# bcsefercik/markerless-robot-camera-calibration

Measured on AMD Instinct MI355X. Metric: point-cloud frames/sec at 200k pts/frame, higher is better.
Workload: dtype f32

## Files before the change

### markerless-robot-camera-calibration_amd/csrc/sv_conv.hip

```cpp
#include <stdarg.h>
#include <stdio.h>
#include <stdlib.h>
#include <vector>

#include "sv_conv_params.h"

namespace sv {

static thread_local char g_last_instance[128] = "";
static thread_local double g_want_scale_override = -1.0;
static thread_local double g_tail_override = -1.0;
void note_instance(const char* fmt, ...) {
  va_list ap;
  va_start(ap, fmt);
  vsnprintf(g_last_instance, sizeof(g_last_instance), fmt, ap);
  va_end(ap);
}
#ifndef SV_CONV_WANT_SCALE_DEFAULT
#define SV_CONV_WANT_SCALE_DEFAULT 0.3
#endif
#ifndef SV_CONV_TAIL_DEFAULT
#define SV_CONV_TAIL_DEFAULT 0.15
#endif
constexpr int chunk_for(int tm, int waves_n) {
// ... 482 lines not shown
  const int rc = launch_traced(q, grid.x, TM_, WAVES_N, NT, stream, [&] {
    if (F && fast && full) {
      if (ring)
        hipLaunchKernelGGL((conv_fwd_kernel<TM_, WAVES_N, NT, F, CPO, (Cfg::PFD > 1), (F && Cfg::USE_FULL)>), grid, dim3(256), lds, stream, q);
      else
        hipLaunchKernelGGL((conv_fwd_kernel<TM_, WAVES_N, NT, F, CPO, false, (F && Cfg::USE_FULL)>), grid, dim3(256), lds, stream, q);
    } else if (F && fast) {
      if (ring)
        hipLaunchKernelGGL((conv_fwd_kernel<TM_, WAVES_N, NT, F, CPO, (Cfg::PFD > 1)>), grid, dim3(256), lds, stream, q);
      else
        hipLaunchKernelGGL((conv_fwd_kernel<TM_, WAVES_N, NT, F, CPO, false>), grid, dim3(256), lds, stream, q);
    } else {
      if (ring)
        hipLaunchKernelGGL((conv_fwd_kernel<TM_, WAVES_N, NT, false, CPO, (Cfg::PFD > 1)>), grid, dim3(256), lds, stream, q);
      else
        hipLaunchKernelGGL((conv_fwd_kernel<TM_, WAVES_N, NT, false, CPO, false>), grid, dim3(256), lds, stream, q);
    }
  });
  if (rc != SV_OK) return rc;
  {
    const bool f = F && fast;
    if (CPO)
      note_instance("conv_fwd_kernel<%d, %d, %d, fused %d>|fast=%d,ring=%d,full=%d", TM_, WAVES_N, NT, CPO, (int)f, (int)ring,
                    (int)(f && full));
    else
      note_instance("conv_fwd_kernel<%d, %d, %d>|fast=%d,ring=%d,full=%d", TM_, WAVES_N, NT, (int)f, (int)ring, (int)(f && full));
  }
  return SV_OK;
}

template <int TM_, int TAIL_TM, int WAVES_N, int NT>
static int launch_conv_dual(const ConvParams& p, hipStream_t stream, double tail_fraction) {
  using Main = ConvCfg<TM_, WAVES_N, NT, 0>;
  using Tail = ConvCfg<TAIL_TM, WAVES_N, NT, 0>;
  const bool fast = p.vec_a && p.buf_ok && (p.Cout % Main::TN == 0);
  const int n128 = (int)(p.Vpad / PLAN_TILE);
  const int tail128 = (int)(n128 * tail_fraction);
  if (!fast || !p.tile_order || tail128 < 1 || tail128 >= n128) return SV_ERR_INVALID;
  ConvParams q = p;
  q.ny = p.Cout / Main::TN;
  q.main_tiles128 = n128 - tail128;
  q.main_blocks = q.main_tiles128 * (PLAN_TILE / TM_) * q.ny;
  q.ntiles = (int)(p.Vpad / TM_);
  const unsigned grid = (unsigned)(q.main_blocks + tail128 * (PLAN_TILE / TAIL_TM) * q.ny);
  const size_t lds = Main::lds_bytes(p.K) > Tail::lds_bytes(p.K) ? Main::lds_bytes(p.K) : Tail::lds_bytes(p.K);
  const int rc = launch_traced(q, grid, TM_, WAVES_N, NT, stream, [&] {
    hipLaunchKernelGGL((conv_fwd_dual_kernel<TM_, TAIL_TM, WAVES_N, NT, true>), dim3(grid), dim3(256), lds, stream, q);
  });
  if (rc != SV_OK) return rc;
  note_instance("conv_fwd_dual_kernel<%d, %d, %d, %d>|fast=1,ring=0,full=0", TM_, TAIL_TM, WAVES_N, NT);
  return SV_OK;
}

struct Candidate {
  int tm, wn, nt;
  int64_t want;
  int cpo;
};

template <int TM_, int WAVES_N, int NT, int CPO = 0>
static bool try_launch(const Candidate& c, const ConvParams& p, hipStream_t stream, int& rc) {
  if (c.tm == TM_ && c.wn == WAVES_N && c.nt == NT && c.cpo == CPO) {
    rc = launch_conv<TM_, WAVES_N, NT, CPO>(p, stream);
    return true;
  }
  return false;
}

static int launch_candidate(const Candidate& c, const ConvParams& p, hipStream_t stream) {
  int rc = SV_ERR_INVALID;
  if (try_launch<128, 4, 3>(c, p, stream, rc) || try_launch<128, 2, 3>(c, p, stream, rc) ||
      try_launch<128, 1, 3>(c, p, stream, rc) || try_launch<64, 4, 3>(c, p, stream, rc) ||
      try_launch<64, 2, 3>(c, p, stream, rc) || try_launch<64, 1, 3>(c, p, stream, rc) ||
      try_launch<32, 4, 3>(c, p, stream, rc) || try_launch<32, 2, 3>(c, p, stream, rc) ||
      try_launch<16, 4, 3>(c, p, stream, rc) ||
      try_launch<128, 4, 2>(c, p, stream, rc) || try_launch<128, 2, 2>(c, p, stream, rc) ||
      try_launch<128, 1, 2>(c, p, stream, rc) || try_launch<64, 4, 2>(c, p, stream, rc) ||
      try_launch<64, 2, 2>(c, p, stream, rc) || try_launch<64, 1, 2>(c, p, stream, rc) ||
      try_launch<32, 4, 2>(c, p, stream, rc) || try_launch<32, 2, 2>(c, p, stream, rc) ||
      try_launch<16, 4, 2>(c, p, stream, rc) ||
      try_launch<64, 4, 1>(c, p, stream, rc) || try_launch<32, 4, 1>(c, p, stream, rc) ||
      try_launch<16, 4, 1>(c, p, stream, rc) || try_launch<128, 2, 1>(c, p, stream, rc) ||
      try_launch<64, 2, 1>(c, p, stream, rc) || try_launch<32, 2, 1>(c, p, stream, rc) ||
      try_launch<128, 1, 1>(c, p, stream, rc) || try_launch<64, 1, 1>(c, p, stream, rc) ||
      try_launch<64, 2, 1, 3>(c, p, stream, rc) || try_launch<32, 2, 1, 3>(c, p, stream, rc) ||
      try_launch<64, 2, 1, 32>(c, p, stream, rc) || try_launch<32, 2, 1, 32>(c, p, stream, rc) ||
      try_launch<32, 4, 1, 32>(c, p, stream, rc) || try_launch<16, 4, 1, 32>(c, p, stream, rc) ||
      try_launch<32, 4, 1, 64>(c, p, stream, rc) || try_launch<16, 4, 1, 64>(c, p, stream, rc))
    return rc;
  set_error("sv_conv_fwd: no kernel instance <%d,%d,%d> cpo %d", c.tm, c.wn, c.nt, c.cpo);
  return SV_ERR_INVALID;
}

static int64_t candidate_wgs(const Candidate& c, const ConvParams& p) {
  const int tn = c.wn * c.nt * 16;
  return (p.Vpad / c.tm) * ((p.Cout + tn - 1) / tn);
}

static int select_and_launch(const ConvParams& p, hipStream_t stream) {
  static const Candidate wide3[] = {{64, 4, 3, 2500}, {32, 4, 3, 1500}, {32, 2, 3, 0}};
  static const Candidate wide3_128[] = {{64, 4, 3, 2500}, {64, 4, 2, 1200}, {32, 4, 3, 1200}, {16, 4, 3, 0}};
  static const Candidate wide3_128_full[] = {{64, 4, 3, 2500}, {32, 4, 3, 1200}, {16, 4, 3, 0}};
  static const Candidate wide2[] = {{128, 4, 2, 1300}, {64, 4, 2, 1500}, {32, 4, 2, 1500}, {32, 2, 2, 0}};
  static const Candidate wide2_64[] = {{128, 4, 2, 1300}, {64, 4, 2, 1500}, {32, 4, 2, 1500}, {16, 4, 1, 0}};
  static const Candidate c64[] = {{64, 4, 1, 1500}, {32, 4, 1, 1500}, {16, 4, 1, 0}};
  static const Candidate c32[] = {{128, 2, 1, 1500}, {64, 2, 1, 1500}, {32, 2, 1, 0}};
  static const Candidate c16[] = {{128, 1, 1, 600}, {64, 1, 1, 0}};
  const Candidate* list;
  int n;
  const int Cout = p.Cout;
  if (Cout > 128 && (Cout % 192 == 0 || Cout % 96 == 0 || Cout > 2048)) {
    if (Cout % 128 != 0) { list = wide3; n = 3; }
    else if (p.Cin % 128 == 0 && p.vec_a) { list = wide3_128_full; n = 3; }
    else { list = wide3_128; n = 4; }
  }
  else if (Cout > 64) { list = Cout % 64 == 0 ? wide2_64 : wide2; n = 4; }
  else if (Cout > 32) { list = c64; n = 3; }
  else if (Cout > 16) { list = c32; n = 3; }
  else { list = c16; n = 2; }
  static const Candidate f3[] = {{64, 2, 1, 3000, 3}, {32, 2, 1, 0, 3}};
  static const Candidate f32_32[] = {{64, 2, 1, 3000, 32}, {32, 2, 1, 0, 32}};
  static const Candidate f32_64[] = {{32, 4, 1, 1500, 32}, {16, 4, 1, 0, 32}};
  static const Candidate f64_64[] = {{32, 4, 1, 1500, 64}, {16, 4, 1, 0, 64}};
  if (p.K > 1) {
    if (p.Cin == 3 && Cout > 16 && Cout <= 32) { list = f3; n = 2; }
    else if (p.Cin == 32 && p.vec_a && Cout == 32) { list = f32_32; n = 2; }
    else if (p.Cin == 32 && p.vec_a && Cout == 64) { list = f32_64; n = 2; }
    else if (p.Cin == 64 && p.vec_a && (Cout == 64 || Cout == 128)) { list = f64_64; n = 2; }
  }
  if (const char* f = getenv("SV_CONV_FORCE_RANGE")) {
    long long vmin = 0, vmax = 0;
    int cout = 0;
    Candidate c = {0, 0, 0, 0, 0};
    if (sscanf(f, "%lld:%lld:%d:%d,%d,%d", &vmin, &vmax, &cout, &c.tm, &c.wn, &c.nt) == 6 && p.Vpad >= vmin && p.Vpad <= vmax &&
        p.Cout == cout && p.K > 1)
      return launch_candidate(c, p, stream);
  }
  if (const char* f = getenv("SV_CONV_FORCE_DENSE")) {
    long long vmin = 0;
    int cout = 0;
    Candidate c = {0, 0, 0, 0, 0};
    if (sscanf(f, "%lld:%d:%d,%d,%d", &vmin, &cout, &c.tm, &c.wn, &c.nt) == 5 && p.Vpad >= vmin && p.Cout == cout && p.K == 1)
      return launch_candidate(c, p, stream);
  }
  if (const char* f = getenv("SV_CONV_FORCE")) {
    Candidate c = {0, 0, 0, 0, 0};
    if (sscanf(f, "%d,%d,%d,%d", &c.tm, &c.wn, &c.nt, &c.cpo) >= 3) return launch_candidate(c, p, stream);
  }
  static const double want_scale =
      getenv("SV_CONV_WANT_SCALE") ? atof(getenv("SV_CONV_WANT_SCALE")) : SV_CONV_WANT_SCALE_DEFAULT;
  static const double tail_fraction = getenv("SV_CONV_TAIL") ? atof(getenv("SV_CONV_TAIL")) : SV_CONV_TAIL_DEFAULT;
  const double ws = g_want_scale_override >= 0.0 ? g_want_scale_override : want_scale;
  const double tf = g_tail_override >= 0.0 ? g_tail_override : tail_fraction;
  for (int i = 0; i < n; ++i)
    if ((double)candidate_wgs(list[i], p) >= ws * (double)list[i].want) {
      const Candidate& c = list[i];
      if (c.tm == 64 && c.wn == 4 && c.nt == 3 && c.cpo == 0 && tf > 0.0 &&
          launch_conv_dual<64, 32, 4, 3>(p, stream, tf) == SV_OK)
        return SV_OK;
      return launch_candidate(c, p, stream);
    }
  return launch_candidate(list[n - 1], p, stream);
}

}

using namespace sv;

extern "C" const char* sv_conv_last_instance(void) { return sv::g_last_instance; }

extern "C" int sv_conv_set_dispatch(double want_scale, double tail_fraction) {
  SV_CHECK_ARG(tail_fraction < 1.0, "tail_fraction must be below 1");
  sv::g_want_scale_override = want_scale;
  sv::g_tail_override = tail_fraction;
  return SV_OK;
}

extern "C" int sv_conv_fwd(const float* in, int64_t V_in, int64_t in_ld, int Cin, const float* W, int K, int Cout,
                           const int32_t* perm, const int32_t* nbr_s, const uint32_t* submask,
                           const int32_t* tile_order, int64_t V_out, int64_t Vpad, const float* scale, const float* shift, const float* residual, int64_t res_ld,
                           int act, float slope, float* out, int64_t out_ld, sv_stream_t stream_) {
  return sv_conv_fwd_acc(in, V_in, in_ld, Cin, W, K, Cout, perm, nbr_s, submask, tile_order, V_out, Vpad, nullptr, 0, scale, shift,
                         residual, res_ld, act, slope, out, out_ld, stream_);
}

extern "C" int sv_conv_fwd_acc(const float* in, int64_t V_in, int64_t in_ld, int Cin, const float* W, int K, int Cout,
                               const int32_t* perm, const int32_t* nbr_s, const uint32_t* submask, const int32_t* tile_order,
                               int64_t V_out, int64_t Vpad, const float* acc_init, int64_t acc_ld, const float* scale,
                               const float* shift, const float* residual, int64_t res_ld, int act, float slope, float* out,
                               int64_t out_ld, sv_stream_t stream_) {
  hipStream_t stream = (hipStream_t)stream_;
  SV_CHECK_ARG(!acc_init || acc_ld >= Cout, "acc_init stride too small");
  SV_CHECK_ARG(Cin > 0 && Cout > 0 && K >= 1 && K <= 32, "bad channel / kernel volume");
  SV_CHECK_ARG(V_out >= 0 && Vpad >= V_out && Vpad % PLAN_TILE == 0, "Vpad must be a multiple of 128 >= V_out");
  SV_CHECK_ARG(in_ld >= Cin && out_ld >= Cout, "row strides too small");
  SV_CHECK_ARG(act >= SV_ACT_NONE && act <= SV_ACT_LEAKY_RELU, "bad activation");
  if (V_out == 0) return SV_OK;
  SV_CHECK_ARG(in && W && out, "null pointer");
  SV_CHECK_ARG(V_in >= 1, "V_in = rows of `in` (every index of the plan is below it)");
  const bool has_plan = perm || nbr_s || submask;
  SV_CHECK_ARG(!has_plan || (perm && nbr_s && submask), "perm, nbr_s and submask must be given together");
  SV_CHECK_ARG(has_plan || K == 1, "K > 1 needs a plan");
  SV_CHECK_ARG(!residual || res_ld >= Cout, "residual stride too small");
  ConvParams p;
  p.in = in; p.in_ld = in_ld; p.Cin = Cin; p.W = W; p.K = K; p.Cout = Cout;
  p.perm = perm; p.nbr_s = nbr_s; p.submask = submask; p.tile_order = tile_order; p.V_out = V_out; p.Vpad = Vpad;
  p.scale = scale; p.shift = shift; p.residual = residual; p.res_ld = res_ld;
  p.acc_init = acc_init; p.acc_ld = acc_ld;
  p.act = act; p.slope = slope; p.out = out; p.out_ld = out_ld;
  p.vec_a = (in_ld % 4 == 0) && (Cin % 4 == 0) && (((uintptr_t)in & 15) == 0);
  const uint64_t in_bytes = ((uint64_t)(V_in - 1) * (uint64_t)in_ld + (uint64_t)Cin) * 4u;
  const uint64_t w_bytes = (uint64_t)K * (uint64_t)Cin * (uint64_t)Cout * 4u;
  const uint64_t out_bytes = ((uint64_t)(V_out - 1) * (uint64_t)out_ld + (uint64_t)Cout) * 4u;
  const uint64_t res_bytes = residual ? ((uint64_t)(V_out - 1) * (uint64_t)res_ld + (uint64_t)Cout) * 4u : 0u;
  const uint64_t acc_bytes = acc_init ? ((uint64_t)(V_out - 1) * (uint64_t)acc_ld + (uint64_t)Cout) * 4u : 0u;
  p.buf_ok = in_bytes < BUF_LIMIT && w_bytes < BUF_LIMIT && out_bytes < BUF_LIMIT && res_bytes < BUF_LIMIT &&
             acc_bytes < BUF_LIMIT && (((uintptr_t)perm & 15) == 0);
  p.acc_bytes = p.buf_ok ? (uint32_t)acc_bytes : 0u;
  if (!p.buf_ok && !has_plan && K == 1 && w_bytes < BUF_LIMIT) {
    int64_t ld_max = in_ld > out_ld ? in_ld : out_ld;
    if (residual && res_ld > ld_max) ld_max = res_ld;
    const int64_t rows = (int64_t)((BUF_LIMIT - 4096u) / ((uint64_t)ld_max * 4u)) / PLAN_TILE * PLAN_TILE;
    if (rows >= PLAN_TILE && rows < V_out) {
      for (int64_t r0 = 0; r0 < V_out; r0 += rows) {
        const int64_t n = V_out - r0 < rows ? V_out - r0 : rows;
        const int rc = sv_conv_fwd_acc(in + r0 * in_ld, n, in_ld, Cin, W, K, Cout, nullptr, nullptr, nullptr, nullptr, n,
                                       (n + PLAN_TILE - 1) / PLAN_TILE * PLAN_TILE, acc_init ? acc_init + r0 * acc_ld : nullptr,
                                       acc_ld, scale, shift, residual ? residual + r0 * res_ld : nullptr, res_ld, act, slope,
                                       out + r0 * out_ld, out_ld, stream_);
        if (rc != SV_OK) return rc;
      }
      return SV_OK;
    }
  }
  p.in_bytes = p.buf_ok ? (uint32_t)in_bytes : 0u;
  p.w_bytes = p.buf_ok ? (uint32_t)w_bytes : 0u;
  p.out_bytes = p.buf_ok ? (uint32_t)out_bytes : 0u;
  p.res_bytes = p.buf_ok ? (uint32_t)res_bytes : 0u;
  p.ntiles = 0;
  p.ny = 0;
  p.trace = nullptr;
  p.main_blocks = 0;
  p.main_tiles128 = 0;
  if (has_plan && K > 1 && K <= 27 && Cin == 3 && Cout == 32 && !acc_init) {
    if (p.buf_ok) return launch_conv_first_mfma(p, stream);
    return launch_conv_first_layer(p, stream);
  }
  if (has_plan && K > 1 && K <= 32 && Cin == 32 && Cout == 32 && p.vec_a && p.buf_ok && !acc_init)
    return launch_conv_thin(p, stream, sv::g_want_scale_override >= 1.0);
  if (!has_plan && K == 1 && Cout <= 4 && p.vec_a && Cin >= 64 && !acc_init) return launch_linear_narrow(p, stream);
  return select_and_launch(p, stream);
}
```

### markerless-robot-camera-calibration_amd/csrc/sv_conv_params.h

```cpp
#pragma once
#include <type_traits>

#include "sv_common.h"

namespace sv {

typedef float f32x4 __attribute__((ext_vector_type(4)));

struct ConvParams {
  const float* in;
  int64_t in_ld;
  int Cin;
  const float* W;
  int K;
  int Cout;
  const int32_t* perm;
  const int32_t* nbr_s;
  const uint32_t* submask;
  const int32_t* tile_order;
  int64_t V_out;
  int64_t Vpad;
  const float* scale;
  const float* shift;
  const float* residual;
  int64_t res_ld;
  const float* acc_init;
  int64_t acc_ld;
  uint32_t acc_bytes;
  int act;
  float slope;
  float* out;
  int64_t out_ld;
  int vec_a;
  uint32_t in_bytes, w_bytes, out_bytes, res_bytes;
  int buf_ok;
  int ntiles;
  int ny;
  unsigned long long* trace;
  int main_blocks;
  int main_tiles128;
};

constexpr int PLAN_TILE = SV_TILE_ROWS;
void note_instance(const char* fmt, ...);
int launch_conv_first_mfma(const ConvParams& p, hipStream_t stream);
int launch_conv_first_layer(const ConvParams& p, hipStream_t stream);
int launch_conv_thin(const ConvParams& p, hipStream_t stream, bool alone);
int launch_linear_narrow(const ConvParams& p, hipStream_t stream);

constexpr uint32_t BUF_ABSENT = 0x80000000u;
constexpr uint32_t BUF_LIMIT = 0x7fff0000u;
typedef int i32x4_t __attribute__((ext_vector_type(4)));
typedef int i32x3_t __attribute__((ext_vector_type(3)));
typedef int i32x2_t __attribute__((ext_vector_type(2)));
template <int N>
__device__ __forceinline__ auto buffer_load_floats(__amdgpu_buffer_rsrc_t rsrc, uint32_t voffset, uint32_t soffset) {
  typedef float vec_t __attribute__((ext_vector_type(N)));
  if constexpr (N == 1) {
    vec_t r;
    r[0] = __builtin_bit_cast(float, __builtin_amdgcn_raw_buffer_load_b32(rsrc, voffset, soffset, 0));
    return r;
  } else if constexpr (N == 2) {
    return __builtin_bit_cast(vec_t, __builtin_amdgcn_raw_buffer_load_b64(rsrc, voffset, soffset, 0));
  } else if constexpr (N == 3) {
    return __builtin_bit_cast(vec_t, __builtin_amdgcn_raw_buffer_load_b96(rsrc, voffset, soffset, 0));
  } else {
    static_assert(N == 4, "1..4 floats per load");
    return __builtin_bit_cast(vec_t, __builtin_amdgcn_raw_buffer_load_b128(rsrc, voffset, soffset, 0));
  }
}

template <int MR>
__device__ __forceinline__ void load_perm_rows(const ConvParams& p, const int64_t rows0, const int lq, int (&o)[MR][4]) {
#pragma unroll
  for (int s = 0; s < MR; ++s) {
    const int64_t r = rows0 + s * 16 + lq * 4;
    if (p.perm) {
      const int4 o4 = *(const int4*)(p.perm + r);
      o[s][0] = o4.x;
      o[s][1] = o4.y;
      o[s][2] = o4.z;
      o[s][3] = o4.w;
    } else {
#pragma unroll
      for (int reg = 0; reg < 4; ++reg) o[s][reg] = (r + reg < p.V_out) ? (int)(r + reg) : -1;
    }
  }
}

template <int MR, int NT, bool PRELOADED = false>
__device__ __forceinline__ void epilogue_buffered(const ConvParams& p, const f32x4 (&acc)[MR][NT], const int64_t rows0,
                                                  const int lq, const int col0, const int (*o_pre)[4] = nullptr) {
  typedef float yvec_t __attribute__((ext_vector_type(NT)));
  const __amdgpu_buffer_rsrc_t rsrc_out = __builtin_amdgcn_make_buffer_rsrc((void*)p.out, 0, (int)p.out_bytes, 0x00020000);
  const __amdgpu_buffer_rsrc_t rsrc_res =
      __builtin_amdgcn_make_buffer_rsrc((void*)p.residual, 0, p.residual ? (int)p.res_bytes : 0, 0x00020000);
  int o[MR][4];
  if constexpr (PRELOADED) {
#pragma unroll
    for (int s = 0; s < MR; ++s)
#pragma unroll
      for (int reg = 0; reg < 4; ++reg) o[s][reg] = o_pre[s][reg];
  } else {
    load_perm_rows<MR>(p, rows0, lq, o);
  }
  float scf[NT], shf[NT];
#pragma unroll
  for (int n = 0; n < NT; ++n) {
    scf[n] = p.scale ? p.scale[col0 + n] : 1.0f;
    shf[n] = p.shift ? p.shift[col0 + n] : (p.scale ? 0.0f : -0.0f);
  }
  const float slope = p.slope;
  auto finish = [&](auto act_tag) {
    constexpr int ACT = decltype(act_tag)::value;
#pragma unroll
    for (int s = 0; s < MR; ++s) {
      yvec_t res[4];
#pragma unroll
      for (int reg = 0; reg < 4; ++reg)
#pragma unroll
        for (int n = 0; n < NT; ++n) res[reg][n] = -0.0f;
      if (p.residual) {
#pragma unroll
        for (int reg = 0; reg < 4; ++reg)
          res[reg] = buffer_load_floats<NT>(
              rsrc_res, o[s][reg] >= 0 ? (uint32_t)o[s][reg] * (uint32_t)(p.res_ld * 4) + (uint32_t)col0 * 4u : BUF_ABSENT,
              0u);
      }
#pragma unroll
      for (int reg = 0; reg < 4; ++reg) {
        yvec_t y;
#pragma unroll
        for (int n = 0; n < NT; ++n) {
          float v = __builtin_fmaf(acc[s][n][reg], scf[n], shf[n]) + res[reg][n];
          if constexpr (ACT == SV_ACT_RELU)
            v = v < 0.f ? 0.f : v;
          else if constexpr (ACT == SV_ACT_LEAKY_RELU)
            v = v > 0.f ? v : v * slope;
          y[n] = v;
        }
        const uint32_t off =
            o[s][reg] >= 0 ? (uint32_t)o[s][reg] * (uint32_t)(p.out_ld * 4) + (uint32_t)col0 * 4u : BUF_ABSENT;
        if constexpr (NT == 1)
          __builtin_amdgcn_raw_buffer_store_b32(__builtin_bit_cast(int, y[0]), rsrc_out, off, 0, 0);
        else if constexpr (NT == 2)
          __builtin_amdgcn_raw_buffer_store_b64(__builtin_bit_cast(i32x2_t, y), rsrc_out, off, 0, 0);
        else if constexpr (NT == 3)
          __builtin_amdgcn_raw_buffer_store_b96(__builtin_bit_cast(i32x3_t, y), rsrc_out, off, 0, 0);
        else
          __builtin_amdgcn_raw_buffer_store_b128(__builtin_bit_cast(i32x4_t, y), rsrc_out, off, 0, 0);
      }
    }
  };
  if (p.act == SV_ACT_RELU)
    finish(std::integral_constant<int, SV_ACT_RELU>{});
  else if (p.act == SV_ACT_LEAKY_RELU)
    finish(std::integral_constant<int, SV_ACT_LEAKY_RELU>{});
  else
    finish(std::integral_constant<int, SV_ACT_NONE>{});
}

}
```

### markerless-robot-camera-calibration_amd/nn.py

```python
import math
from ctypes import c_float, c_int, c_int64, c_size_t

import numpy as np
import torch
import torch.nn as nn

from . import _lib, profiling
from ._lib import SV_ACT_LEAKY_RELU, SV_ACT_NONE, SV_ACT_RELU, call, ptr, stream_ptr
from .sparse import SparseTensor, SplitPlan

KERNEL_OFFSET_PERMUTATION = None

import os as _os


def _parse_split_rules(text):
    rules = []
    for part in text.split(";"):
        if part.strip():
            rows, _, cuts = part.partition(":")
            cuts = tuple(int(v) for v in cuts.split(",") if v)
            rules.append((int(rows), cuts[0] if len(cuts) == 1 else cuts))
    return sorted(rules, key=lambda r: -r[0])


SPLIT_RULES = _parse_split_rules(_os.environ.get("MRCC_SPLIT_RULES", "20000:9,18"))
SPLIT_MIN_CHANNELS = int(_os.environ.get("MRCC_SPLIT_MIN_CHANNELS", "128"))


SPLIT_RULES_ONE_FRAME = _parse_split_rules(_os.environ.get("MRCC_SPLIT_RULES_ONE_FRAME", "50000:9,18"))


def split_points_for(rows):
    for min_rows, cuts in SPLIT_RULES:
        if rows >= min_rows:
            return cuts
    return None


def conv_forward(feats, weight3, plan, V_out, scale=None, shift=None, residual=None, act=SV_ACT_NONE, slope=0.01,
                 out=None, weight_bf16=None):
    K, Cin, Cout = weight3.shape
    if feats.shape[1] != Cin:
        raise ValueError(f"input has {feats.shape[1]} channels, kernel expects {Cin}")
    if feats.stride(1) != 1:
        feats = feats.contiguous()
    if out is None:
        out = torch.empty((V_out, Cout), dtype=torch.float32, device=feats.device)
    if isinstance(plan, SplitPlan):
        return _conv_forward_split(feats, weight3, plan, V_out, scale, shift, residual, act, slope, out, weight_bf16)
    return _conv_forward_one(feats, weight3, plan, V_out, scale, shift, residual, act, slope, out, None, wp=weight_bf16)


def pack_weights_bf16(weight3):
    K, Cin, Cout = weight3.shape
    w = weight3.detach().float().contiguous()
    wp = torch.empty(K * Cin * Cout, dtype=torch.bfloat16, device=w.device)
    call("sv_pack_weights_bf16", ptr(w), c_int(K), c_int(Cin), c_int(Cout), ptr(wp), stream_ptr())
    return wp


def _conv_forward_split(feats, weight3, plan, V_out, scale, shift, residual, act, slope, out, weight_bf16=None):
    K, Cin, Cout = weight3.shape
    timer = profiling.TIMER
    t0 = None
    if timer is not None:
        kname = profiling.conv_kernel_config(Cout, plan.Vpad, Cin, plan.parts[-1][1] - plan.parts[-1][0])
        if timer.want(kname):
            t0 = timer.start()
    if weight_bf16 is None and not weight3.is_contiguous():
        weight3 = weight3.contiguous()
    acc = None
    for i, (k0, k1, sub) in enumerate(plan.parts):
        w = weight3[k0:k1]
        wp = weight_bf16[k0 * Cin * Cout:k1 * Cin * Cout] if weight_bf16 is not None else None
        if i == len(plan.parts) - 1:
            _conv_forward_one(feats, w, sub, V_out, scale, shift, residual, act, slope, out, acc, timed=False, wp=wp)
        else:
            nxt = torch.empty((V_out, Cout), dtype=torch.float32, device=feats.device)
            _conv_forward_one(feats, w, sub, V_out, None, None, None, SV_ACT_NONE, slope, nxt, acc, timed=False, wp=wp)
            acc = nxt
    if t0 is not None:
        timer.stop(t0, _lib.conv_last_instance()[0], K, Cin, Cout, V_out, plan.pairs_device(), level=plan.out_stride,
                   passes=len(plan.parts))
    return out


def _conv_forward_one(feats, weight3, plan, V_out, scale, shift, residual, act, slope, out, acc_init, timed=True, wp=None):
    K, Cin, Cout = weight3.shape
    if plan is None:
        Vpad = (max(V_out, 1) + _lib.SV_TILE_ROWS - 1) // _lib.SV_TILE_ROWS * _lib.SV_TILE_ROWS
    else:
        Vpad = plan.Vpad
    timer = profiling.TIMER if timed else None
    t0 = None
    if timer is not None:
        kname = profiling.conv_kernel_config(Cout, Vpad, Cin, K)
        if timer.want(kname):
            t0 = timer.start()
    res_ld = residual.stride(0) if residual is not None else 0

    log = profiling.INSTANCE_LOG

    acc_ld = acc_init.stride(0) if acc_init is not None else 0

    fn, w_arg = ("sv_conv_fwd_acc", weight3) if wp is None else ("sv_conv_fwd_bf16", wp)

    def launch(f, pl, o, r, v_out, v_pad, a=None):
        call(fn, ptr(f), c_int64(f.shape[0]), c_int64(f.stride(0)), c_int(Cin), ptr(w_arg), c_int(K),
             c_int(Cout), ptr(pl.perm if pl else None), ptr(pl.nbr_s if pl else None), ptr(pl.submask if pl else None),
             ptr(pl.tile_order if pl else None), c_int64(v_out), c_int64(v_pad), ptr(a), c_int64(acc_ld), ptr(scale), ptr(shift),
             ptr(r), c_int64(res_ld), c_int(act), c_float(slope), ptr(o), c_int64(o.stride(0)), stream_ptr())
        if log is not None:
            log.append((*_lib.conv_last_instance(), K, Cin, Cout, v_out))

    parts = plan.chunks(4 * feats.stride(0), 4 * max(out.stride(0), res_ld, acc_ld)) if plan is not None else None
    if parts is None:
        launch(feats, plan, out, residual, V_out, Vpad, acc_init)
    else:
        for sub, i0, i1, o0, o1 in parts:
            launch(feats[i0:i1], sub, out[o0:o1], residual[o0:o1] if residual is not None else None, o1 - o0, sub.Vpad,
                   acc_init[o0:o1] if acc_init is not None else None)
    if t0 is not None:
        timer.stop(t0, _lib.conv_last_instance()[0], K, Cin, Cout, V_out,
                   plan.pairs_device() if plan is not None else None,
                   level=plan.out_stride if plan is not None else None)
    return out


def _wgrad_one(feats, dy, plan, K, Cin, Cout, V_out, dW, accumulate, bf16=False):
    Vpad = (plan.Vpad if plan is not None
            else (max(V_out, 1) + _lib.SV_TILE_ROWS - 1) // _lib.SV_TILE_ROWS * _lib.SV_TILE_ROWS)
    lib = _lib.load()
    fn = "sv_conv_wgrad_bf16" if bf16 else "sv_conv_wgrad"
    nbytes = getattr(lib, fn + "_workspace_bytes")(c_int64(Vpad), c_int(K), c_int(Cin), c_int(Cout))
    ws = torch.empty(max(nbytes, 1), dtype=torch.uint8, device=dy.device)
    rc = getattr(lib, fn)(ptr(feats), c_int64(feats.shape[0]), c_int64(feats.stride(0)), c_int(Cin), ptr(dy),
                          c_int64(V_out), c_int64(dy.stride(0)), c_int(Cout), c_int(K), ptr(plan.perm if plan else None),
                          ptr(plan.nbr_s if plan else None), ptr(plan.submask if plan else None), c_int64(Vpad),
                          c_int(1 if accumulate else 0), ptr(ws), c_size_t(nbytes), ptr(dW), stream_ptr())
    if bf16 and rc == _lib.SV_ERR_UNSUPPORTED:
        return _wgrad_one(feats, dy, plan, K, Cin, Cout, V_out, dW, accumulate)
    _lib._check(rc, fn)
    return fn


def conv_wgrad(feats, dy, plan, K, Cin, Cout, bf16=False, used=None):
    if feats.stride(1) != 1:
        feats = feats.contiguous()
    if dy.stride(1) != 1:
        dy = dy.contiguous()
    V_out = dy.shape[0]
    dW = torch.empty((K, Cin, Cout), dtype=torch.float32, device=dy.device)
    used = set() if used is None else used
    if isinstance(plan, SplitPlan):
        for k0, k1, sub in plan.parts:
            _wgrad_plan(feats, dy, sub, k1 - k0, Cin, Cout, V_out, dW[k0:k1], bf16, used)
    else:
        _wgrad_plan(feats, dy, plan, K, Cin, Cout, V_out, dW, bf16, used)
    return dW


def _wgrad_plan(feats, dy, plan, K, Cin, Cout, V_out, dW, bf16=False, used=None):
    used = set() if used is None else used
    parts = plan.chunks(4 * feats.stride(0), 4 * dy.stride(0)) if plan is not None else None
    if parts is None:
        used.add(_wgrad_one(feats, dy, plan, K, Cin, Cout, V_out, dW, False, bf16))
        return
    for j, (sub, i0, i1, o0, o1) in enumerate(parts):
        used.add(_wgrad_one(feats[i0:i1], dy[o0:o1], sub, K, Cin, Cout, o1 - o0, dW, j > 0, bf16))


def _bf16_fwd_ok(rows, Cin, Cout, K):
    return (Cin % 32 == 0 and Cin >= 64 and Cout % 16 == 0 and Cout >= 64 and K <= 27
            and rows.data_ptr() % 16 == 0 and rows.stride(0) % 4 == 0)


def _train_log(layer, op, fn):
    log = profiling.TRAIN_LOG
    if log is not None:
        log.append((layer, op, fn))


class SparseConvFunction(torch.autograd.Function):

    @staticmethod
    def forward(ctx, feats, weight3, bias, plan, V_out, grad_plan, mirror, layer=None):
        w = weight3.detach()
        if not w.is_contiguous():
            w = w.contiguous()
        bf16 = layer is not None and hasattr(layer, "_train_bf16") and layer._train_bf16()
        shift = bias.detach().reshape(-1) if bias is not None else None
        wp = layer.packed_weights_bf16() if bf16 and _bf16_fwd_ok(feats, w.shape[1], w.shape[2], w.shape[0]) else None
        out = conv_forward(feats.detach(), w, plan, V_out, None, shift, weight_bf16=wp)
        _train_log(layer, "fwd", "sv_conv_fwd_acc" if wp is None else "sv_conv_fwd_bf16")
        ctx.save_for_backward(feats, w)
        ctx.plan, ctx.grad_plan, ctx.mirror, ctx.layer, ctx.bf16 = plan, grad_plan, mirror, layer, bf16
        ctx.bias_shape = bias.shape if bias is not None else None
        return out

    @staticmethod
    def backward(ctx, dy):
        feats, w = ctx.saved_tensors
        K, Cin, Cout = w.shape
        if dy.stride(1) != 1:
            dy = dy.contiguous()
        dx = dw = db = None
        if ctx.needs_input_grad[0]:
            if ctx.bf16 and _bf16_fwd_ok(dy, Cout, Cin, K) and (Cin % 128 == 0 or Cin % 192 == 0):
                dx = conv_forward(dy, w.transpose(1, 2), ctx.grad_plan(), feats.shape[0],
                                  weight_bf16=ctx.layer.packed_grad_weights_bf16(ctx.mirror))
                _train_log(ctx.layer, "dx", "sv_conv_fwd_bf16")
            else:
                wt = (w.flip(0) if ctx.mirror else w).transpose(1, 2).contiguous()
                dx = conv_forward(dy, wt, ctx.grad_plan(), feats.shape[0])
                _train_log(ctx.layer, "dx", "sv_conv_fwd_acc")
        if ctx.needs_input_grad[1]:
            used = set()
            dw = conv_wgrad(feats.detach(), dy, ctx.plan, K, Cin, Cout, bf16=ctx.bf16, used=used)
            _train_log(ctx.layer, "dw", "+".join(sorted(used)))
        if ctx.bias_shape is not None and ctx.needs_input_grad[2]:
            db = dy.sum(0).reshape(ctx.bias_shape)
        return dx, dw, db, None, None, None, None, None


def sparse_conv(feats, weight3, bias, plan, V_out, grad_plan, mirror=False, layer=None):
    return SparseConvFunction.apply(feats, weight3, bias, plan, V_out, grad_plan, mirror, layer)


def _act_torch(x, act, slope):
    if act == SV_ACT_RELU:
        return torch.relu(x)
    if act == SV_ACT_LEAKY_RELU:
        return torch.nn.functional.leaky_relu(x, slope)
    return x


def linear_train(linear, x, act=SV_ACT_NONE, slope=0.01, layer=None):
    if x.stride(1) != 1:
        x = x.contiguous()
    out = sparse_conv(x, linear.weight.t().unsqueeze(0), linear.bias, None, x.shape[0], lambda: None, layer=layer)
    return _act_torch(out, act, slope)


def affine_act(feats, scale=None, shift=None, residual=None, act=SV_ACT_NONE, slope=0.01):
    V, C = feats.shape
    if feats.stride(1) != 1:
        feats = feats.contiguous()
    out = torch.empty((V, C), dtype=torch.float32, device=feats.device)
    call("sv_affine_act", ptr(feats), c_int64(feats.stride(0)), c_int(C), c_int64(V), ptr(scale), ptr(shift),
# ... 447 lines not shown
```

### markerless-robot-camera-calibration_amd/profiling.py

```python
import math

import torch

TIMER = None
INSTANCE_LOG = None
TRAIN_LOG = None

_CANDIDATES = {
    "wide3": [(64, 4, 3, 2500), (32, 4, 3, 1500), (32, 2, 3, 0)],
    "wide3_128": [(64, 4, 3, 2500), (64, 4, 2, 1200), (32, 4, 3, 1200), (16, 4, 3, 0)],
    "wide3_128_full": [(64, 4, 3, 2500), (32, 4, 3, 1200), (16, 4, 3, 0)],
    "wide2": [(128, 4, 2, 1300), (64, 4, 2, 1500), (32, 4, 2, 1500), (32, 2, 2, 0)],
    "wide2_64": [(128, 4, 2, 1300), (64, 4, 2, 1500), (32, 4, 2, 1500), (16, 4, 1, 0)],
    "c64": [(64, 4, 1, 1500), (32, 4, 1, 1500), (16, 4, 1, 0)],
    "c32": [(128, 2, 1, 1500), (64, 2, 1, 1500), (32, 2, 1, 0)],
    "c16": [(128, 1, 1, 600), (64, 1, 1, 0)],
}


import os

CONV_TAIL_FRACTION = float(os.environ.get("SV_CONV_TAIL", "0.15"))
CONV_WANT_SCALE = float(os.environ.get("SV_CONV_WANT_SCALE", "0.3"))


_FUSED = {
    (32, 32): [(64, 2, 1, 3000), (32, 2, 1, 0)],
    (32, 64): [(32, 4, 1, 1500), (16, 4, 1, 0)],
    (64, 64): [(32, 4, 1, 1500), (16, 4, 1, 0)],
    (64, 128): [(32, 4, 1, 1500), (16, 4, 1, 0)],
}


def conv_kernel_config(Cout, Vpad, Cin=None, K=1):
    if K == 1 and Cout <= 4 and Cin is not None and Cin >= 64 and Cin % 4 == 0:
        return f"linear_narrow_kernel<{Cout}>"
    if K > 1 and Cin == 3 and Cout == 32:
        return "conv_first_mfma_kernel<3, 32>"
    if K > 1 and Cin == 32 and Cout == 32:
        return "conv_thin_kernel<32, 32>"
    fused = None
    if K > 1 and Cin is not None:
        if Cin == 3 and 16 < Cout <= 32:
            fused = [(64, 2, 1, 3000), (32, 2, 1, 0)]
        else:
            fused = _FUSED.get((Cin, Cout))
    if fused is not None:
        cands = fused
    elif Cout > 128 and (Cout % 192 == 0 or Cout % 96 == 0 or Cout > 2048):
        if Cout % 128 != 0:
            cands = _CANDIDATES["wide3"]
        else:
            cands = _CANDIDATES["wide3_128_full" if (Cin is not None and Cin % 128 == 0) else "wide3_128"]
    elif Cout > 64:
        cands = _CANDIDATES["wide2_64" if Cout % 64 == 0 else "wide2"]
    elif Cout > 32:
        cands = _CANDIDATES["c64"]
    elif Cout > 16:
        cands = _CANDIDATES["c32"]
    else:
        cands = _CANDIDATES["c16"]
    suffix = f", fused {Cin}>" if fused is not None else ">"
    for tm, wn, nt, want in cands:
        tn = wn * nt * 16
        if (Vpad // tm) * ((Cout + tn - 1) // tn) >= want * CONV_WANT_SCALE:
            if ((tm, wn, nt) == (64, 4, 3) and fused is None and K > 1 and Cin is not None and Cin % 4 == 0
                    and Cout % tn == 0 and CONV_TAIL_FRACTION > 0 and int((Vpad // 128) * CONV_TAIL_FRACTION) >= 1):
                return "conv_fwd_dual_kernel<64, 32, 4, 3>"
            return f"conv_fwd_kernel<{tm}, {wn}, {nt}{suffix}"
    tm, wn, nt, _ = cands[-1]
    return f"conv_fwd_kernel<{tm}, {wn}, {nt}{suffix}"


class KernelTimer:
    def __init__(self, capacity=0):
        self.records = []
        self.enabled = True
        self.only = None
        self._pool = [torch.cuda.Event(enable_timing=True) for _ in range(capacity)]
        self._next = 0
        self._first_of_frame = False

    def _event(self):
        if self._next < len(self._pool):
            e = self._pool[self._next]
            self._next += 1
            return e
        return torch.cuda.Event(enable_timing=True)

    def want(self, kernel):
        return self.enabled and (self.only is None or kernel in self.only)

    def start(self):
        e = self._event()
        e.record()
        return e

    def stop(self, start_evt, kernel, K, Cin, Cout, V_out, pairs_dev, level=None, passes=1):
        e = self._event()
        e.record()
        self.records.append((kernel, K, Cin, Cout, V_out, pairs_dev, start_evt, e, self._first_of_frame, level, passes))
        self._first_of_frame = False

    def frame_boundary(self):
        self._first_of_frame = True

    def clear(self):
        self.records = []

    @staticmethod
    def layer_key(kernel, K, Cin, Cout, V_out, level=None):
        where = f"s{level}" if level is not None else f"~2^{int(round(math.log2(max(V_out, 1))))}"
        return (kernel, K, Cin, Cout, where)

    def summarize(self, by_layer=False):
        out = {}
        for kernel, K, Cin, Cout, V_out, pairs_dev, s, e, first, level, passes in self.records:
            if first:
                continue
            P = int(pairs_dev.item()) if pairs_dev is not None else V_out
            ms = s.elapsed_time(e)
            key = self.layer_key(kernel, K, Cin, Cout, V_out, level) if by_layer else kernel
            d = out.setdefault(key, {"launches": 0, "ms": 0.0, "flops": 0.0, "bytes": 0.0, "rows": 0.0, "kernel_launches": 0})
            d["rows"] += V_out
            d["launches"] += 1
            d["kernel_launches"] += passes
            d["ms"] += ms
            d["flops"] += 2.0 * P * Cin * Cout
            d["bytes"] += P * (4.0 * Cin + 8) + 4.0 * V_out * Cout + 4.0 * K * Cin * Cout
        return out


def pass_gflop(fn):
    global TIMER
    saved, TIMER = TIMER, KernelTimer()
    try:
        fn()
        torch.cuda.synchronize()
        return sum(d["flops"] for d in TIMER.summarize().values()) / 1e9
    finally:
        TIMER = saved
```

Before: 73.64.

## Add dense persistent 1x1 conv kernel with multi-tile workgroups and double-buffered LDS

Adds a specialised kernel for pointwise (K=1, no permutation) convolutions that reads input rows directly, double-buffers input chunks in LDS, and processes several row tiles per workgroup. Each tile's epilogue is overlapped with the next tile's loads. It is chosen by default when a candidate shape is eligible, with the tiles per workgroup sized from the workgroup count. The aim is to cut gather/permutation overhead and per-workgroup setup for dense 1x1 layers, at the cost of fewer workgroups and added register and LDS pressure.

```diff
diff --git a/markerless-robot-camera-calibration_amd/csrc/sv_conv.hip b/markerless-robot-camera-calibration_amd/csrc/sv_conv.hip
--- a/markerless-robot-camera-calibration_amd/csrc/sv_conv.hip
+++ b/markerless-robot-camera-calibration_amd/csrc/sv_conv.hip
@@ -658,9 +658,17 @@
   static const double tail_fraction = getenv("SV_CONV_TAIL") ? atof(getenv("SV_CONV_TAIL")) : SV_CONV_TAIL_DEFAULT;
   const double ws = g_want_scale_override >= 0.0 ? g_want_scale_override : want_scale;
   const double tf = g_tail_override >= 0.0 ? g_tail_override : tail_fraction;
+  const char* dense_env = getenv("SV_CONV_DENSE_TILES");
+  const int dense_tiles = dense_env ? atoi(dense_env) : -1;
+  if (dense_tiles > 0 && conv_dense_eligible(p, list[0].tm, list[0].wn, list[0].nt))
+    return launch_conv_dense(p, stream, list[0].tm, dense_tiles);
   for (int i = 0; i < n; ++i)
     if ((double)candidate_wgs(list[i], p) >= ws * (double)list[i].want) {
       const Candidate& c = list[i];
+      if (dense_tiles != 0 && conv_dense_eligible(p, c.tm, c.wn, c.nt)) {
+        const int64_t per_wg = candidate_wgs(c, p) / 2560;
+        return launch_conv_dense(p, stream, c.tm, (int)(per_wg < 1 ? 1 : (per_wg > DENSE_MAX_TILES ? DENSE_MAX_TILES : per_wg)));
+      }
       if (c.tm == 64 && c.wn == 4 && c.nt == 3 && c.cpo == 0 && tf > 0.0 &&
           launch_conv_dual<64, 32, 4, 3>(p, stream, tf) == SV_OK)
         return SV_OK;
diff --git a/markerless-robot-camera-calibration_amd/csrc/sv_conv_dense.hip b/markerless-robot-camera-calibration_amd/csrc/sv_conv_dense.hip
--- /dev/null
+++ b/markerless-robot-camera-calibration_amd/csrc/sv_conv_dense.hip
@@ -0,0 +1,203 @@
+#include "sv_conv_params.h"
+
+namespace sv {
+
+constexpr int DENSE_KC = 32;
+constexpr int DENSE_SA = 34;
+
+template <int TM_, int NT>
+__global__ __launch_bounds__(256) __attribute__((amdgpu_waves_per_eu(4, 4))) void conv_dense_kernel(ConvParams p, int tiles_per_wg) {
+  constexpr int KC = DENSE_KC, SA = DENSE_SA, KS = KC / 4;
+  constexpr int MR = TM_ / 16;
+  constexpr int TN = 4 * NT * 16;
+  constexpr int ROWS_PER_PASS = 256 / (KC / 4);
+  constexpr int A_F4 = TM_ / ROWS_PER_PASS;
+  static_assert(TM_ % ROWS_PER_PASS == 0, "whole passes of 32 rows");
+  extern __shared__ __attribute__((aligned(16))) float lds[];
+  typedef float bvec_t __attribute__((ext_vector_type(NT)));
+
+  const int tid = threadIdx.x;
+  const int lane = tid & 63;
+  const int wn = __builtin_amdgcn_readfirstlane(tid >> 6);
+  const int li = lane & 15, lq = lane >> 4;
+  const int ny = p.Cout / TN;
+  const int n0 = ((int)blockIdx.x % ny) * TN;
+  const int tile0 = ((int)blockIdx.x / ny) * tiles_per_wg;
+  const int ntile = min(tiles_per_wg, p.ntiles - tile0);
+  const int Cout = p.Cout;
+  const int nchunks = p.Cin / KC;
+  const int col0 = n0 + wn * NT * 16 + NT * li;
+
+  const __amdgpu_buffer_rsrc_t rsrc_in = __builtin_amdgcn_make_buffer_rsrc((void*)p.in, 0, (int)p.in_bytes, 0x00020000);
+  const __amdgpu_buffer_rsrc_t rsrc_w = __builtin_amdgcn_make_buffer_rsrc((void*)p.W, 0, (int)p.w_bytes, 0x00020000);
+  const __amdgpu_buffer_rsrc_t rsrc_out = __builtin_amdgcn_make_buffer_rsrc((void*)p.out, 0, (int)p.out_bytes, 0x00020000);
+  const __amdgpu_buffer_rsrc_t rsrc_res =
+      __builtin_amdgcn_make_buffer_rsrc((void*)p.residual, 0, p.residual ? (int)p.res_bytes : 0, 0x00020000);
+
+  const int a_cc = (tid % (KC / 4)) * 4;
+  const int a_r = tid / (KC / 4);
+  uint32_t a_off;
+  const uint32_t pass_bytes = (uint32_t)ROWS_PER_PASS * (uint32_t)(p.in_ld * 4);
+  auto first_tile = [&]() { a_off = ((uint32_t)tile0 * TM_ + (uint32_t)a_r) * (uint32_t)(p.in_ld * 4) + (uint32_t)a_cc * 4u; };
+  auto next_tile = [&](int t) { a_off = t < ntile ? a_off + (uint32_t)TM_ * (uint32_t)(p.in_ld * 4) : BUF_ABSENT; };
+  float4 ra[A_F4];
+  auto load_a = [&](int c0) {
+#pragma unroll
+    for (int j = 0; j < A_F4; ++j) {
+      const f32x4 v = buffer_load_floats<4>(rsrc_in, a_off, (uint32_t)c0 * 4u + (uint32_t)j * pass_bytes);
+      ra[j] = make_float4(v[0], v[1], v[2], v[3]);
+    }
+  };
+  auto store_a = [&](float* dstbuf) {
+#pragma unroll
+    for (int j = 0; j < A_F4; ++j) {
+      float2* dst = (float2*)(dstbuf + (a_r + ROWS_PER_PASS * j) * SA + a_cc);
+      dst[0] = make_float2(ra[j].x, ra[j].y);
+      dst[1] = make_float2(ra[j].z, ra[j].w);
+    }
+  };
+  bvec_t b[KS];
+  const uint32_t b_off_bytes = (uint32_t)(lq * Cout + col0) * 4u;
+  auto load_b = [&](int c0, int ks) { b[ks] = buffer_load_floats<NT>(rsrc_w, b_off_bytes, (uint32_t)(c0 + 4 * ks) * (uint32_t)Cout * 4u); };
+
+  float scf[NT], shf[NT];
+#pragma unroll
+  for (int n = 0; n < NT; ++n) {
+    scf[n] = p.scale ? p.scale[col0 + n] : 1.0f;
+    shf[n] = p.shift ? p.shift[col0 + n] : (p.scale ? 0.0f : -0.0f);
+  }
+  const float slope = p.slope;
+  const int act = p.act;
+  const int v_out = (int)p.V_out;
+  auto flush_sub = [&](const f32x4 (&a)[NT], const int r0) {
+    const int nrow = v_out - r0;
+    bvec_t res[4];
+#pragma unroll
+    for (int reg = 0; reg < 4; ++reg)
+#pragma unroll
+      for (int n = 0; n < NT; ++n) res[reg][n] = -0.0f;
+    if (p.residual) {
+#pragma unroll
+      for (int reg = 0; reg < 4; ++reg)
+        res[reg] = buffer_load_floats<NT>(
+            rsrc_res, reg < nrow ? (uint32_t)(r0 + reg) * (uint32_t)(p.res_ld * 4) + (uint32_t)col0 * 4u : BUF_ABSENT, 0u);
+    }
+    auto finish = [&](auto act_tag) {
+      constexpr int ACT = decltype(act_tag)::value;
+#pragma unroll
+      for (int reg = 0; reg < 4; ++reg) {
+        bvec_t y;
+#pragma unroll
+        for (int n = 0; n < NT; ++n) {
+          float v = __builtin_fmaf(a[n][reg], scf[n], shf[n]) + res[reg][n];
+          if constexpr (ACT == SV_ACT_RELU)
+            v = v < 0.f ? 0.f : v;
+          else if constexpr (ACT == SV_ACT_LEAKY_RELU)
+            v = v > 0.f ? v : v * slope;
+          y[n] = v;
+        }
+        const uint32_t off = reg < nrow ? (uint32_t)(r0 + reg) * (uint32_t)(p.out_ld * 4) + (uint32_t)col0 * 4u : BUF_ABSENT;
+        if constexpr (NT == 2)
+          __builtin_amdgcn_raw_buffer_store_b64(__builtin_bit_cast(i32x2_t, y), rsrc_out, off, 0, 0);
+        else
+          __builtin_amdgcn_raw_buffer_store_b96(__builtin_bit_cast(i32x3_t, y), rsrc_out, off, 0, 0);
+      }
+    };
+    if (act == SV_ACT_RELU)
+      finish(std::integral_constant<int, SV_ACT_RELU>{});
+    else if (act == SV_ACT_LEAKY_RELU)
+      finish(std::integral_constant<int, SV_ACT_LEAKY_RELU>{});
+    else
+      finish(std::integral_constant<int, SV_ACT_NONE>{});
+  };
+  static_assert(NT == 2 || NT == 3, "the two dense tile shapes");
+
+  f32x4 acc[MR][NT];
+#pragma unroll
+  for (int s = 0; s < MR; ++s)
+#pragma unroll
+    for (int n = 0; n < NT; ++n) acc[s][n] = (f32x4){0.f, 0.f, 0.f, 0.f};
+
+  first_tile();
+  load_a(0);
+#pragma unroll
+  for (int ks = 0; ks < KS; ++ks) load_b(0, ks);
+  store_a(lds);
+  __syncthreads();
+  int buf = 0;
+
+  auto step = [&](const int cx, const int flush_rows) {
+    load_a(cx);
+    if (flush_rows >= 0) {
+#pragma unroll
+      for (int s = 0; s < MR; ++s) {
+        flush_sub(acc[s], flush_rows + s * 16 + lq * 4);
+#pragma unroll
+        for (int n = 0; n < NT; ++n) acc[s][n] = (f32x4){0.f, 0.f, 0.f, 0.f};
+        __builtin_amdgcn_sched_barrier(0);
+      }
+    }
+    const float* a_base = lds + buf * (TM_ * SA) + li * SA + lq;
+    float a[MR];
+#pragma unroll
+    for (int s = 0; s < MR; ++s) a[s] = a_base[s * 16 * SA];
+#pragma unroll
+    for (int ks = 0; ks < KS; ++ks) {
+#pragma unroll
+      for (int s = 0; s < MR; ++s) {
+#pragma unroll
+        for (int n = 0; n < NT; ++n) acc[s][n] = __builtin_amdgcn_mfma_f32_16x16x4f32(a[s], b[ks][n], acc[s][n], 0, 0, 0);
+        if (ks + 1 < KS) a[s] = a_base[s * 16 * SA + (ks + 1) * 4];
+        __builtin_amdgcn_sched_barrier(0);
+      }
+      load_b(cx, ks);
+      __builtin_amdgcn_sched_barrier(0);
+    }
+  };
+
+  for (int t = 0; t < ntile; ++t) {
+    const int rows_before = t > 0 ? (tile0 + t - 1) * TM_ : -1;
+    for (int c = 0; c < nchunks; ++c) {
+      const bool last = c + 1 == nchunks;
+      if (last) next_tile(t + 1);
+      step(last ? 0 : (c + 1) * KC, c == 0 ? rows_before : -1);
+      if (last && t + 1 == ntile) break;
+      store_a(lds + (buf ^ 1) * (TM_ * SA));
+      __syncthreads();
+      buf ^= 1;
+    }
+  }
+  const int rows_last = (tile0 + ntile - 1) * TM_;
+#pragma unroll
+  for (int s = 0; s < MR; ++s) flush_sub(acc[s], rows_last + s * 16 + lq * 4);
+}
+
+template <int TM_, int NT>
+static int launch_dense(const ConvParams& p, hipStream_t stream, int tiles_per_wg) {
+  constexpr int TN = 4 * NT * 16;
+  ConvParams q = p;
+  q.ntiles = (int)(p.Vpad / TM_);
+  q.ny = p.Cout / TN;
+  const unsigned grid = (unsigned)((q.ntiles + tiles_per_wg - 1) / tiles_per_wg * q.ny);
+  const size_t lds = (size_t)2 * TM_ * DENSE_SA * sizeof(float);
+  hipLaunchKernelGGL((conv_dense_kernel<TM_, NT>), dim3(grid), dim3(256), lds, stream, q, tiles_per_wg);
+  SV_LAUNCH_CHECK();
+  note_instance("conv_dense_kernel<%d, 4, %d>|fast=1,ring=0,full=1,tiles=%d", TM_, NT, tiles_per_wg);
+  return SV_OK;
+}
+
+bool conv_dense_eligible(const ConvParams& p, int tm, int wn, int nt) {
+  if (!((tm == 128 && wn == 4 && nt == 2) || (tm == 64 && wn == 4 && nt == 3))) return false;
+  return p.K == 1 && !p.perm && !p.acc_init && p.vec_a && p.buf_ok && p.Cout > 4 && p.Cout % (wn * nt * 16) == 0 &&
+         p.Cin % DENSE_KC == 0 && (uint64_t)p.Vpad * (uint64_t)p.in_ld * 4u < 0xf0000000ull;
+}
+
+int launch_conv_dense(const ConvParams& p, hipStream_t stream, int tm, int tiles_per_wg) {
+  if (tiles_per_wg < 1 || tiles_per_wg > DENSE_MAX_TILES) {
+    set_error("sv_conv_fwd: dense body takes 1..%d row tiles per workgroup, not %d", DENSE_MAX_TILES, tiles_per_wg);
+    return SV_ERR_INVALID;
+  }
+  return tm == 128 ? launch_dense<128, 2>(p, stream, tiles_per_wg) : launch_dense<64, 3>(p, stream, tiles_per_wg);
+}
+
+}
diff --git a/markerless-robot-camera-calibration_amd/csrc/sv_conv_params.h b/markerless-robot-camera-calibration_amd/csrc/sv_conv_params.h
--- a/markerless-robot-camera-calibration_amd/csrc/sv_conv_params.h
+++ b/markerless-robot-camera-calibration_amd/csrc/sv_conv_params.h
@@ -47,6 +47,9 @@
 int launch_conv_first_layer(const ConvParams& p, hipStream_t stream);
 int launch_conv_thin(const ConvParams& p, hipStream_t stream, bool alone);
 int launch_linear_narrow(const ConvParams& p, hipStream_t stream);
+constexpr int DENSE_MAX_TILES = 4;
+bool conv_dense_eligible(const ConvParams& p, int tm, int wn, int nt);
+int launch_conv_dense(const ConvParams& p, hipStream_t stream, int tm, int tiles_per_wg);
 
 constexpr uint32_t BUF_ABSENT = 0x80000000u;
 constexpr uint32_t BUF_LIMIT = 0x7fff0000u;
diff --git a/markerless-robot-camera-calibration_amd/nn.py b/markerless-robot-camera-calibration_amd/nn.py
--- a/markerless-robot-camera-calibration_amd/nn.py
+++ b/markerless-robot-camera-calibration_amd/nn.py
@@ -95,7 +95,7 @@
     timer = profiling.TIMER if timed else None
     t0 = None
     if timer is not None:
-        kname = profiling.conv_kernel_config(Cout, Vpad, Cin, K)
+        kname = profiling.conv_kernel_config(Cout, Vpad, Cin, K, body=True, plan=plan is not None)
         if timer.want(kname):
             t0 = timer.start()
     res_ld = residual.stride(0) if residual is not None else 0
diff --git a/markerless-robot-camera-calibration_amd/profiling.py b/markerless-robot-camera-calibration_amd/profiling.py
--- a/markerless-robot-camera-calibration_amd/profiling.py
+++ b/markerless-robot-camera-calibration_amd/profiling.py
@@ -32,7 +32,21 @@
 }
 
 
-def conv_kernel_config(Cout, Vpad, Cin=None, K=1):
+CONV_DENSE_TILES = int(os.environ.get("SV_CONV_DENSE_TILES", "-1"))
+
+
+def conv_dense_tiles(tm, wn, nt, Cout, Vpad, Cin, K, plan=False, forced=False):
+    tn = wn * nt * 16
+    if (K != 1 or plan or Cin is None or Cin % 32 or Cout <= 4 or Cout % tn or (tm, wn, nt) not in ((128, 4, 2), (64, 4, 3))
+            or CONV_DENSE_TILES == 0):
+        return 0
+    if forced:
+        return max(CONV_DENSE_TILES, 0)
+    return min(max((Vpad // tm) * (Cout // tn) // 2560, 1), 4)
+
+
+def conv_kernel_config(Cout, Vpad, Cin=None, K=1, body=False, plan=None):
+    has_plan = (K > 1) if plan is None else bool(plan)
     if K == 1 and Cout <= 4 and Cin is not None and Cin >= 64 and Cin % 4 == 0:
         return f"linear_narrow_kernel<{Cout}>"
     if K > 1 and Cin == 3 and Cout == 32:
@@ -61,9 +75,13 @@
     else:
         cands = _CANDIDATES["c16"]
     suffix = f", fused {Cin}>" if fused is not None else ">"
+    if body and CONV_DENSE_TILES > 0 and conv_dense_tiles(*cands[0][:3], Cout, Vpad, Cin, K, has_plan, forced=True):
+        return "conv_dense_kernel<%d, %d, %d>" % cands[0][:3]
     for tm, wn, nt, want in cands:
         tn = wn * nt * 16
         if (Vpad // tm) * ((Cout + tn - 1) // tn) >= want * CONV_WANT_SCALE:
+            if body and conv_dense_tiles(tm, wn, nt, Cout, Vpad, Cin, K, has_plan):
+                return f"conv_dense_kernel<{tm}, {wn}, {nt}>"
             if ((tm, wn, nt) == (64, 4, 3) and fused is None and K > 1 and Cin is not None and Cin % 4 == 0
                     and Cout % tn == 0 and CONV_TAIL_FRACTION > 0 and int((Vpad // 128) * CONV_TAIL_FRACTION) >= 1):
                 return "conv_fwd_dual_kernel<64, 32, 4, 3>"
```

Result: no change. 73.64, median of 3 (-0.0%).
